# qitianwu/SGFormer

Measured on AMD Instinct MI355X. Metric: SGFormer fwd+bwd nodes/sec on ogbn-products full-graph, higher is better.
Workload: dtype bf16

## Files before the change

include/sgf.h:

```cpp
#ifndef SGF_H_
#define SGF_H_

#include <stddef.h>
#include <stdint.h>

#ifdef __cplusplus
extern "C" {
#endif

#define SGF_VERSION 666

#define SGF_F32 0
#define SGF_BF16 1
#define SGF_F32_BF16X3 2

#define SGF_OK 0
#define SGF_E_INVALID (-1)
#define SGF_E_WORKSPACE (-2)
#define SGF_E_HIP (-3)
#define SGF_E_UNSUPPORTED (-4)

int sgf_version(void);
const char* sgf_last_error(void);
int sgf_reload_env(void);

size_t sgf_csr_workspace_bytes(int64_t nnz, int64_t n);
int sgf_csr_build(const int64_t* edge_index, int64_t nnz, int64_t n, int64_t* rowptr,
                  int32_t* colind, float* val, int32_t* deg, void* workspace,
                  size_t workspace_bytes, void* stream);

int sgf_csr_transpose(const int64_t* edge_index, int64_t nnz, int64_t n, const int32_t* deg,
                      const int64_t* rowptr, const int32_t* colind, int64_t* t_rowptr,
                      int32_t* t_colind, float* t_val, int32_t* is_symmetric, void* workspace,
                      size_t workspace_bytes, void* stream);

size_t sgf_subgraph_workspace_bytes(int64_t nnz, int64_t n);
int sgf_subgraph_plan(const int64_t* edge_index, int64_t nnz, int64_t n, const int64_t* subset,
                      int64_t m, int32_t* relabel, int64_t* total, void* workspace,
                      size_t workspace_bytes, void* stream);
int sgf_subgraph_emit(const int64_t* edge_index, int64_t nnz, int64_t n, const int32_t* relabel,
                      int32_t relabel_nodes, int64_t total, int64_t* out, int64_t* out_eid,
                      void* workspace, size_t workspace_bytes, void* stream);

// ... 353 lines not shown
size_t sgf_argmax_workspace_bytes(int64_t m, int32_t c);
int sgf_argmax_count(const void* logits, int64_t ldl, int64_t n, int32_t c, int32_t dtype, const void* labels,
                     int64_t label_stride, int32_t label_kind, const int64_t* idx, int64_t m, int64_t* counts,
                     void* workspace, size_t workspace_bytes, void* stream);

int32_t sgf_head_rows_supported(int32_t d, int32_t classes, int32_t dtype);
size_t sgf_head_rows_fwd_workspace_bytes(int64_t m);
size_t sgf_head_rows_bwd_workspace_bytes(int64_t m, int32_t d, int32_t classes);
int sgf_head_rows_fwd(const void* x1, int64_t ld1, float a, const void* x2, int64_t ld2, float b, const float* w,
                      const float* bias, int64_t n, int32_t d, int32_t classes, int32_t dtype, const int64_t* idx,
                      int64_t m, float* logits, int64_t ldl, const int64_t* labels, float* lse, float* loss_sum,
                      int64_t* counts, void* workspace, size_t workspace_bytes, void* stream);
int sgf_head_rows_bwd(const void* x1, int64_t ld1, float a, const void* x2, int64_t ld2, float b, const float* w,
                      int64_t n, int32_t d, int32_t classes, int32_t dtype, const int64_t* idx, int64_t m,
                      const float* dlogits, int64_t lddl, const float* logits, int64_t ldl, const float* lse,
                      const int64_t* labels, const float* gout, float inv_denom, void* dx1, int64_t ldd1, void* dx2,
                      int64_t ldd2, float* dw, float* db, void* workspace, size_t workspace_bytes, void* stream);

int32_t sgf_pair_sigmoid_supported(int32_t heads, int32_t v_heads, int32_t d, int32_t dtype);
size_t sgf_pair_sigmoid_workspace_bytes(int64_t n, int64_t l, int32_t heads);
int64_t sgf_pair_sigmoid_lap_rows(int32_t which, int32_t heads, int32_t d, int32_t dtype, int32_t laps);
int sgf_pair_sigmoid_fwd(const void* q, int64_t ldq, const void* k, int64_t ldk, const void* v, int64_t ldv, int64_t n,
                         int64_t l, int32_t heads, int32_t v_heads, int32_t d, int32_t dtype, void* out, int64_t ldo,
                         float* rowsum, void* stream);
int sgf_pair_sigmoid_bwd_q(const void* g, int64_t ldg, const void* out, int64_t ldo, const float* rowsum, const void* q,
                           int64_t ldq, const void* k, int64_t ldk, const void* v, int64_t ldv, int64_t n, int64_t l,
                           int32_t heads, int32_t v_heads, int32_t d, int32_t dtype, void* dq, int64_t lddq, void* workspace,
                           size_t workspace_bytes, void* stream);
int sgf_pair_sigmoid_bwd_kv(const void* g, int64_t ldg, const float* rowsum, const void* q, int64_t ldq, const void* k,
                            int64_t ldk, const void* v, int64_t ldv, int64_t n, int64_t l, int32_t heads, int32_t v_heads,
                            int32_t d, int32_t dtype, void* dk, int64_t lddk, void* dv, int64_t lddv, const void* workspace,
                            size_t workspace_bytes, void* stream);

int sgf_sum_n(const void* const* xs_host, const int64_t* lds_host, int32_t k, int64_t n, int32_t d,
              int32_t dtype, void* y, int64_t ldy, void* stream);

size_t sgf_colsum_workspace_bytes(int64_t n, int32_t d);
int sgf_colsum(const void* x, int64_t ldx, int64_t n, int32_t d, int32_t dtype, float* out,
               void* workspace, size_t workspace_bytes, void* stream);

int32_t sgf_comm_available(void);
int32_t sgf_comm_unique_id_bytes(void);
int sgf_comm_unique_id(void* id_host);
int sgf_comm_create(void** comm_out, int32_t world, int32_t rank, const void* id_host);
int sgf_comm_destroy(void* comm);
int sgf_comm_all_reduce_f32(void* comm, float* buf, int64_t count, void* stream);
int sgf_comm_all_gather(void* comm, const void* send, void* recv, int64_t bytes_per_rank, void* stream);
int sgf_comm_all_to_all(void* comm, const void* send, const int64_t* send_offset_host, const int64_t* send_bytes_host,
                        void* recv, const int64_t* recv_offset_host, const int64_t* recv_bytes_host, void* stream);

#ifdef __cplusplus
}
#endif
#endif
```

sgformer_amd/_lib.py:

```python
from __future__ import annotations

import ctypes
import os
from ctypes import c_char_p, c_double, c_float, c_int32, c_int64, c_size_t, c_uint64, c_void_p

_HERE = os.path.dirname(os.path.abspath(__file__))
LIB_PATH = os.path.join(_HERE, "lib", "libsgf.so")

SGF_F32 = 0
SGF_BF16 = 1
SGF_F32_BF16X3 = 2
SGF_OK = 0
SGF_E_INVALID = -1
SGF_E_WORKSPACE = -2
SGF_E_HIP = -3
SGF_E_UNSUPPORTED = -4
SGF_BCE_TARGET_F32 = 0
SGF_BCE_TARGET_I64 = 1
SGF_BCE_TARGET_CLASS = 2
SGF_METRIC_TARGET_F32 = 0
SGF_METRIC_TARGET_I64 = 1

_lib = None

# ... 144 lines not shown
                                  c_int64, _P]),
    "sgf_nll_workspace_bytes": (c_size_t, [c_int64]),
    "sgf_nll_fwd": (c_int32, [_P, c_int64, c_int64, c_int32, c_int32, _P, _P, c_int64, _P, _P, c_size_t, _P]),
    "sgf_nll_bwd": (c_int32, [_P, c_int64, c_int64, c_int32, c_int32, _P, _P, c_int64, _P, c_float, _P,
                              c_int64, _P]),
    "sgf_bce_workspace_bytes": (c_size_t, [c_int64, c_int32]),
    "sgf_bce_fwd": (c_int32, [_P, c_int64, c_int64, c_int32, c_int32, _P, c_int64, c_int32, _P, c_int64, c_float, _P, _P,
                              c_size_t, _P]),
    "sgf_bce_bwd": (c_int32, [_P, c_int64, c_int64, c_int32, c_int32, _P, c_int64, c_int32, _P, c_int64, _P, c_float, _P,
                              c_int64, _P]),
    "sgf_rocauc_workspace_bytes": (c_size_t, [c_int64, c_int32]),
    "sgf_rocauc_counts": (c_int32, [_P, c_int64, c_int64, c_int32, c_int32, _P, c_int64, c_int32, _P, c_int64, _P, _P,
                                    c_size_t, _P]),
    "sgf_argmax_workspace_bytes": (c_size_t, [c_int64, c_int32]),
    "sgf_argmax_count": (c_int32, [_P, c_int64, c_int64, c_int32, c_int32, _P, c_int64, c_int32, _P, c_int64, _P, _P,
                                   c_size_t, _P]),
    "sgf_head_rows_supported": (c_int32, [c_int32, c_int32, c_int32]),
    "sgf_head_rows_fwd_workspace_bytes": (c_size_t, [c_int64]),
    "sgf_head_rows_bwd_workspace_bytes": (c_size_t, [c_int64, c_int32, c_int32]),
    "sgf_head_rows_fwd": (c_int32, [_P, c_int64, c_float, _P, c_int64, c_float, _P, _P, c_int64, c_int32, c_int32, c_int32,
                                    _P, c_int64, _P, c_int64, _P, _P, _P, _P, _P, c_size_t, _P]),
    "sgf_head_rows_bwd": (c_int32, [_P, c_int64, c_float, _P, c_int64, c_float, _P, c_int64, c_int32, c_int32, c_int32,
                                    _P, c_int64, _P, c_int64, _P, c_int64, _P, _P, _P, c_float, _P, c_int64, _P, c_int64,
                                    _P, _P, _P, c_size_t, _P]),
    "sgf_pair_sigmoid_supported": (c_int32, [c_int32, c_int32, c_int32, c_int32]),
    "sgf_pair_sigmoid_workspace_bytes": (c_size_t, [c_int64, c_int64, c_int32]),
    "sgf_pair_sigmoid_lap_rows": (c_int64, [c_int32, c_int32, c_int32, c_int32, c_int32]),
    "sgf_pair_sigmoid_fwd": (c_int32, [_P, c_int64, _P, c_int64, _P, c_int64, c_int64, c_int64, c_int32, c_int32, c_int32,
                                       c_int32, _P, c_int64, _P, _P]),
    "sgf_pair_sigmoid_bwd_q": (c_int32, [_P, c_int64, _P, c_int64, _P, _P, c_int64, _P, c_int64, _P, c_int64, c_int64,
                                         c_int64, c_int32, c_int32, c_int32, c_int32, _P, c_int64, _P, c_size_t, _P]),
    "sgf_pair_sigmoid_bwd_kv": (c_int32, [_P, c_int64, _P, _P, c_int64, _P, c_int64, _P, c_int64, c_int64, c_int64, c_int32,
                                          c_int32, c_int32, c_int32, _P, c_int64, _P, c_int64, _P, c_size_t, _P]),
    "sgf_sum_n": (c_int32, [_P, _P, c_int32, c_int64, c_int32, c_int32, _P, c_int64, _P]),
    "sgf_colsum_workspace_bytes": (c_size_t, [c_int64, c_int32]),
    "sgf_colsum": (c_int32, [_P, c_int64, c_int64, c_int32, c_int32, _P, _P, c_size_t, _P]),
    "sgf_combine_fc_supported": (c_int32, [c_int32, c_int32, c_int32]),
    "sgf_combine_fc_fwd": (c_int32, [_P, c_int64, c_float, _P, c_int64, c_float, _P, _P, c_int64, c_int32, c_int32,
                                     c_int32, _P, c_int64, _P]),
    "sgf_combine_fc_bwd": (c_int32, [_P, c_int64, _P, c_int64, c_int32, c_int32, c_float, c_float, c_int32, _P,
                                     c_int64, _P, c_int64, _P]),
    "sgf_combine_fc_fwd_mapped": (c_int32, [_P, c_int64, c_float, _P, c_int64, c_float, _P, _P, c_int64, c_int32, c_int32,
                                     c_int32, _P, c_int64, _P, _P]),
    "sgf_combine_fc_bwd_g": (c_int32, [_P, c_int64, _P, c_int64, c_int32, c_int32, c_float, c_float, c_int32, _P, c_int64, _P,
                                       c_int64, _P, _P, c_int64, _P]),
    "sgf_combine_fc_bwd_mapped": (c_int32, [_P, c_int64, _P, c_int64, c_int32, c_int32, c_float, c_float, c_int32, _P,
                                     c_int64, _P, c_int64, _P, _P]),
    "sgf_gcn_epilogue_supported": (c_int32, [c_int32, c_int32, c_int32]),
    "sgf_gcn_epilogue_workspace_bytes": (c_size_t, [c_int64, c_int32]),
    "sgf_gcn_epilogue_stats": (c_int32, [_P, c_int64, _P, c_int64, _P, c_int64, c_int32, c_int32, c_int32, _P, c_int64,
                                         _P, _P, _P, c_size_t, _P]),
    "sgf_gcn_epilogue_dx": (c_int32, [_P, c_int64, _P, c_int64, c_int64, c_int32, c_int32, c_int32, _P, c_int64, _P]),
    "sgf_gcn_epilogue_dx2": (c_int32, [_P, c_int64, _P, _P, c_int64, c_int64, c_int32, c_int32, _P, c_int64, _P, c_int64,
                                       c_int32, _P]),
    "sgf_gcn_epilogue_dx2_acc_supported": (c_int32, [c_int32, c_int32]),
    "sgf_gcn_epilogue_dx2_acc": (c_int32, [_P, c_int64, _P, c_int64, c_int64, c_int32, c_int32, _P, c_int64, _P, c_int64, _P,
                                           c_int64, _P, c_int64, _P]),
    "sgf_gcn_epilogue_apply": (c_int32, [_P, c_int64, _P, _P, _P, _P, _P, c_int64, c_int32, c_int64, c_int32,
                               c_int32, _P, c_int64, _P]),
    "sgf_gcn_bn_bwd_dx_supported": (c_int32, [c_int32, c_int32]),
    "sgf_gcn_bn_bwd_dx_workspace_bytes": (c_size_t, [c_int64, c_int32]),
    "sgf_gcn_bn_bwd_dx": (c_int32, [_P, c_int64, _P, c_int64, _P, _P, _P, _P, c_int32, _P, c_float, c_int32, _P, c_int64,
                                    c_int64, c_int32, c_int32, _P, c_int64, _P, c_int64, _P, _P, c_size_t, _P, c_int64,
                                    c_int32, _P, c_size_t, _P]),
    "sgf_gcn_epilogue_cat_supported": (c_int32, [c_int32, c_int32]),
    "sgf_gcn_epilogue_cat": (c_int32, [_P, c_int64, _P, c_int64, _P, c_int64, _P, c_int64, c_int32, c_int32, _P, c_int64,
# ... 62 lines not shown
```

sgformer_amd/csrc/fused.hip:

```cpp
#include "common.h"

namespace sgf {
namespace {

constexpr int kThreads = 256;
constexpr int kMaxD = 1024;
constexpr int kMaxStatBlocks = 2048;

__device__ __forceinline__ float4 zero4() { return make_float4(0.f, 0.f, 0.f, 0.f); }
__device__ __forceinline__ float4 ld4f(const float* p) { return *reinterpret_cast<const float4*>(p); }

inline int lanes_per_row(int d) {
  int l = 16;
  while (l * 4 < d && l < 64) l <<= 1;
  return l;
}

template <typename T, int LPR, int NC>
__global__ __launch_bounds__(kThreads) void k_ln_fwd(
    const T* __restrict__ x, int64_t ldx, const T* __restrict__ res, int64_t ldr, float a, float b,
    const float* __restrict__ gamma, const float* __restrict__ beta, int relu, float eps, int64_t n,
    int d, T* __restrict__ y, int64_t ldy, float* __restrict__ mean, float* __restrict__ rstd) {
  constexpr int RPB = kThreads / LPR;
  const int sl = threadIdx.x % LPR;
// ... 831 lines not shown
      }
    };
    int64_t row = r0 + sr;
    for (; row + (U - 1) * static_cast<int64_t>(rpp) < r1; row += U * static_cast<int64_t>(rpp)) {
      uint4 xv[U], gv[U], hv[U];
#pragma unroll
      for (int u = 0; u < U; ++u) {
        const int64_t rr = row + u * static_cast<int64_t>(rpp);
        xv[u] = *reinterpret_cast<const uint4*>(x + rr * ldx + col);
        gv[u] = *reinterpret_cast<const uint4*>(dy + rr * lddy + col);
        if (kTwo) hv[u] = *reinterpret_cast<const uint4*>(dy2 + rr * lddy2 + col);
      }
#pragma unroll
      for (int u = 0; u < U; ++u) add_row(xv[u], gv[u], kTwo ? hv[u] : gv[u]);
    }
    for (; row < r1; row += rpp) {
      const uint4 xr = *reinterpret_cast<const uint4*>(x + row * ldx + col);
      const uint4 gr = *reinterpret_cast<const uint4*>(dy + row * lddy + col);
      const uint4 hr = kTwo ? *reinterpret_cast<const uint4*>(dy2 + row * lddy2 + col) : gr;
      add_row(xr, gr, hr);
    }
  }
#pragma unroll
  for (int e = 0; e < 8; ++e) {
    red[(0 * kThreads + threadIdx.x) * 8 + e] = s0[e];
    red[(1 * kThreads + threadIdx.x) * 8 + e] = s1[e];
  }
  __syncthreads();
  for (int j = threadIdx.x; j < 2 * d; j += kThreads) {
    const int which = j / d, cc = j % d;
    float s = 0.f;
    for (int r = 0; r < rpp; ++r) s += red[(which * kThreads + r * f8 + cc / 8) * 8 + (cc & 7)];
    part[static_cast<int64_t>(blockIdx.x) * 2 * d + j] = s;
  }
}

template <typename T>
__global__ __launch_bounds__(kThreads) void k_axpby(const T* __restrict__ x1, int64_t ld1, float a,
                                                    const T* __restrict__ x2, int64_t ld2, float b,
                                                    int64_t n, int d, T* __restrict__ y,
                                                    int64_t ldy) {
  const int f4 = d / 4;
  const int64_t total = n * f4;
  for (int64_t i = static_cast<int64_t>(blockIdx.x) * kThreads + threadIdx.x; i < total;
       i += static_cast<int64_t>(gridDim.x) * kThreads) {
    const int64_t row = i / f4;
    const int col = static_cast<int>(i % f4) * 4;
    const float4 u = load4<T>(x1 + row * ld1 + col);
    const float4 v = load4<T>(x2 + row * ld2 + col);
    store4<T>(y + row * ldy + col,
              make_float4(a * u.x + b * v.x, a * u.y + b * v.y, a * u.z + b * v.z, a * u.w + b * v.w));
  }
}

template <typename TS, typename TD, typename TI>
__global__ __launch_bounds__(kThreads) void k_gather_rows(const TS* __restrict__ src, int64_t lds,
                                                          const TI* __restrict__ idx, int64_t n_out, int d,
                                                          int64_t n_src, TD* __restrict__ dst, int64_t ldd,
                                                          int vec) {
  if (vec) {
    const int f4 = d / 4;
    const int64_t total = n_out * f4;
    for (int64_t i = static_cast<int64_t>(blockIdx.x) * kThreads + threadIdx.x; i < total;
         i += static_cast<int64_t>(gridDim.x) * kThreads) {
      const int64_t row = i / f4;
      const int col = static_cast<int>(i % f4) * 4;
// ... 599 lines not shown
}

extern "C" int sgf_bn_bwd_stats(const void* dy, int64_t lddy, const void* x, int64_t ldx,
                                const float* mean, const float* rstd, const float* gamma,
                                const float* beta, int32_t relu, int64_t n, int32_t d,
                                int32_t dtype, float* stats, void* workspace,
                                size_t workspace_bytes, void* stream) {
  return sgf_bn_bwd_stats2(dy, lddy, nullptr, 0, x, ldx, mean, rstd, gamma, beta, relu, n, d, dtype, stats, workspace,
                           workspace_bytes, stream);
}

extern "C" int sgf_bn_bwd_apply(const void* dy, int64_t lddy, const void* x, int64_t ldx,
                                const float* mean, const float* rstd, const float* gamma,
                                const float* beta, int32_t relu, const float* stats, float inv_n,
                                int32_t training, int64_t n, int32_t d, int32_t dtype, void* dx,
                                int64_t lddx, void* stream) {
  int rc = check_ew("sgf_bn_bwd_apply", n, d, dtype);
  if (rc != SGF_OK || n == 0) return rc;
  SGF_REQUIRE(dy && x && dx && mean && rstd && (!training || stats), SGF_E_INVALID,
              "sgf_bn_bwd_apply: null pointer");
  SGF_REQUIRE(lddy % 4 == 0 && ldx % 4 == 0 && lddx % 4 == 0, SGF_E_INVALID,
              "sgf_bn_bwd_apply: leading dims must be multiples of 4");
  hipStream_t st = static_cast<hipStream_t>(stream);
  const BnParams p{mean, rstd, gamma, beta};
  if (dtype == SGF_BF16 && ew8_rows(d, {{dy, lddy}, {x, ldx}, {dx, lddx}}))
    return launch(k_bn_bwd_apply_bf16x8<kEw8Unroll>, dim3(rowwalk8_grid(n, d)), st, dy, lddy, x, ldx, p, relu, stats, inv_n,
                  training, n, d, dx, lddx);
  return by_dtype(dtype, [&](auto t) {
    return launch(k_bn_bwd_apply<decltype(t)>, dim3(rowwalk_grid(n, d)), st, dy, lddy, x, ldx, p, relu, stats, inv_n, training,
                  n, d, dx, lddx);
  });
}

extern "C" int sgf_axpby(const void* x1, int64_t ld1, float a, const void* x2, int64_t ld2, float b,
                         int64_t n, int32_t d, int32_t dtype, void* y, int64_t ldy, void* stream) {
  int rc = check_ew("sgf_axpby", n, d, dtype);
  if (rc != SGF_OK || n == 0) return rc;
  SGF_REQUIRE(x1 && x2 && y && ld1 % 4 == 0 && ld2 % 4 == 0 && ldy % 4 == 0, SGF_E_INVALID,
              "sgf_axpby: bad pointer / ld");
  hipStream_t st = static_cast<hipStream_t>(stream);
  return by_dtype(dtype, [&](auto t) {
    return launch(k_axpby<decltype(t)>, dim3(ew_grid(n * (d / 4))), st, x1, ld1, a, x2, ld2, b, n, d, y, ldy);
  });
}

extern "C" int sgf_gather_rows(const void* src, int64_t lds, int32_t src_dtype, int64_t n_src, const void* idx,
                               int32_t idx_is_int64, int64_t n_out, int32_t d, void* dst, int64_t ldd,
                               int32_t dst_dtype, void* stream) {
  SGF_REQUIRE(n_out >= 0 && d >= 0 && n_src >= 0, SGF_E_INVALID, "sgf_gather_rows: negative size");
  SGF_REQUIRE((src_dtype == SGF_F32 || src_dtype == SGF_BF16) && (dst_dtype == SGF_F32 || dst_dtype == SGF_BF16),
              SGF_E_INVALID, "sgf_gather_rows: unknown dtype");
  if (n_out == 0 || d == 0) return SGF_OK;
  SGF_REQUIRE(src && idx && dst && lds >= d && ldd >= d, SGF_E_INVALID, "sgf_gather_rows: bad pointer / ld");
  const size_t es = src_dtype == SGF_BF16 ? 2 : 4, ed = dst_dtype == SGF_BF16 ? 2 : 4;
  const int vec = d % 4 == 0 && lds % 4 == 0 && ldd % 4 == 0 && reinterpret_cast<uintptr_t>(src) % (4 * es) == 0 &&
                  reinterpret_cast<uintptr_t>(dst) % (4 * ed) == 0;
  hipStream_t st = static_cast<hipStream_t>(stream);
  const dim3 grid(ew_grid(vec ? n_out * (d / 4) : n_out * d));
  return by_copy_types(src_dtype, dst_dtype, idx_is_int64, [&](auto ts, auto td, auto ti) {
    return launch(k_gather_rows<decltype(ts), decltype(td), decltype(ti)>, grid, st, src, lds, idx, n_out, d, n_src, dst, ldd,
                  vec);
  });
}

namespace sgf {
namespace {
// ... 170 lines not shown
```

sgformer_amd/linear.py:

```python
from __future__ import annotations

import os
from functools import partial
from typing import NamedTuple, Optional

import torch
import torch.nn.functional as F

from .kernels import _pair_gram, _rows, _rows16

_F32 = torch.float32
_BF16 = torch.bfloat16

from .graph import K, _has


def _f32c(t):
    return None if t is None else t.detach().float().contiguous()


def _switch(name: str, default: bool) -> bool:
    v = os.environ.get(name)
    return default if v is None else (v != "0" if default else v == "1")

# ... 307 lines not shown

def gcn_layer_fused_ok(x0: torch.Tensor, w: torch.Tensor) -> bool:
    d = x0.shape[1] if x0.dim() == 2 else 0
    return (x0.dim() == 2 and x0.shape[0] > 0 and x0.dtype == _BF16 and tuple(w.shape) == (d, 2 * d)
            and _has(K, "gcn_bn_bwd_dx_supported", d, x0.dtype) and _switch("SGF_GCN_FUSED", True))


class _LinearBNActRes(torch.autograd.Function):

    @staticmethod
    def forward(ctx, y, x0, w, b, gamma, beta, book, relu: bool, use_res: bool, shard, chain, first: bool, pack=None):
        K.check(y, x0)
        dt = x0.dtype
        wc = w.detach().to(dt).contiguous()
        yr, xr = _rows16(y), _rows16(x0)
        z, mean, rstd, n_tot, training = _batchnorm_of(book, partial(_streaming_linear, [yr, xr], wc, _f32c(b)), wc.shape[0],
                                                       yr.shape[0], yr.device, shard)
        g32, be32 = _f32c(gamma), _f32c(beta)
        if pack is not None:
            out, pack["out"] = K.bn_apply_packed(z, mean, rstd, g32, be32, xr if use_res else None, relu, pack["slot_bytes"])
        else:
            out = K.bn_apply(z, mean, rstd, g32, be32, xr if use_res else None, relu)
        ctx.save_for_backward(yr, xr, z, wc, g32, be32, mean, rstd)
        ctx.meta = (bool(relu), bool(use_res), bool(training), float(n_tot), shard, chain, bool(first), w.dtype,
                    None if b is None else b.dtype, None if gamma is None else gamma.dtype)
        return out

    @staticmethod
    def backward(ctx, gout):
        yr, xr, z, wc, g32, be32, mean, rstd = ctx.saved_tensors
        relu, use_res, training, n_tot, shard, chain, first, wdt, bdt, gdt = ctx.meta
        d = z.shape[1]
        gout = _rows16(gout.contiguous())
        stats = K.bn_bwd_stats(gout, z, mean, rstd, g32, be32, relu)
        if shard is not None:
            shard.all_reduce(stats)
        inv_n = 1.0 / max(n_tot, 1.0)
        if _fused_bwd():
            dz, dy, acc = K.gcn_bn_bwd_dx(gout, z, mean, rstd, g32, be32, relu, stats, inv_n, training, wc, chain.acc,
                                          last=first, add_gy=use_res)
            chain.acc = None if first else acc
            dx0 = acc if first else None
        else:
            fused_dw = None
            if ctx.needs_input_grad[2] and _pair_gram() and _has(K, "gram2_bn_bwd_supported", gout, z, yr, xr):
                dwf = torch.empty((d, 2 * d), dtype=_F32, device=z.device)
                dz, dbf = K.gram2_bn_bwd(gout, z, mean, rstd, g32, be32, relu, stats, inv_n, training, yr, xr, dwf[:, :d], dwf[:, d:])
                fused_dw = (dwf.to(wdt), dbf.to(bdt) if (ctx.needs_input_grad[3] and bdt is not None) else None)
            else:
                dz = K.bn_bwd_apply(gout, z, mean, rstd, g32, be32, relu, stats, inv_n, training)
            if _acc_in_place(d, dz.dtype) and not chain.parts:
                dy, chain.acc = K.gcn_epilogue_dx2_acc(dz, wc, _rows16(gout) if use_res else None, chain.acc)
                dx0 = None
                if first:
                    dx0, chain.acc = chain.acc, None
            else:
                dy, dxi = K.gcn_epilogue_dx2(dz, wc[:, :d], wc[:, d:], True)
                chain.parts.append(dxi)
                if use_res:
                    chain.parts.append(gout)
                dx0 = None
                if first:
                    parts, chain.parts = chain.parts, []
                    if chain.acc is not None:
                        parts.append(chain.acc)
                        chain.acc = None
                    dx0 = parts[0] if len(parts) == 1 else (K.sum_n(parts) if len(parts) <= 8 else sum(parts[1:], parts[0]))
        if not _fused_bwd() and fused_dw is not None:
            dw, db = fused_dw
        else:
            dw, db = _linear_param_grads(dz, [yr, xr], [d, d], ctx.needs_input_grad[2],
                                         ctx.needs_input_grad[3] and bdt is not None, wdt, bdt)
        dgamma, dbeta = _bn_param_grads(stats, d, g32, be32, gdt, shard)
        return dy, dx0, dw, db, dgamma, dbeta, None, None, None, None, None, None, None


def linear_bn_act_res(y, x0, w, b, gamma, beta, book, relu, use_res, shard, chain, first, pack=None):
    return _LinearBNActRes.apply(y, x0, w, b, gamma, beta, book, relu, use_res, shard, chain, first, pack)


def _linear(w, b, *xs):
# ... 38 lines not shown
```

sgformer_amd/ops.py:

```python
from __future__ import annotations

from typing import Optional

import torch
import torch.nn.functional as F

from . import kernels as _kernels
from .kernels import HipKernels, LONG_ROW, _SEGMENT, _workspace
from .kernels import _rows, _rows16

_F32 = torch.float32
_BF16 = torch.bfloat16


from . import graph as _graph
from .graph import *
from .graph import K, graph_cache, _own_block_spmm, _sharded_spmm, _tile_params, _block_shape, _mode
from .linear import _bn_param_grads, _f32c, _has, _switch


def set_kernels(table):
    global K
    prev, K = K, table
    _graph.K = _linear.K = table
    graph_cache.clear()
    return prev


def _require_cuda(*tensors):
    K.check(*tensors)


def _split(qkv, v_ext, heads, d):
    hd = heads * d
    q, k = qkv[:, :hd], qkv[:, hd:2 * hd]
    if v_ext is None:
        return q, k, qkv[:, 2 * hd:], heads
    return q, k, v_ext, 1


class _Attention(torch.autograd.Function):

    @staticmethod
    def forward(ctx, qkv, v_ext, heads: int, d: int, shard, n_override=None, per_head=False):
        K.check(qkv, v_ext)
        qkv, v_ext = _rows(qkv), _rows(v_ext)
        n, hd = qkv.shape[0], heads * d
        assert qkv.shape[1] == (3 * hd if v_ext is None else 2 * hd)
        q, k, v, v_heads = _split(qkv, v_ext, heads, d)
        stats = K.attn_fwd_reduce(q, k, v, heads, v_heads, d)
        n_total = float(n) if n_override is None else float(n_override)
        if shard is not None:
            shard.all_reduce(stats)
            if n_override is None:
                n_total = float(shard.n_global)
        out, den, o_heads = K.attn_fwd_apply(q, v, stats, n_total, heads, v_heads, d)
        per_head = bool(per_head) and heads > 1
        ctx.save_for_backward(qkv, v_ext, out, den, o_heads, stats)
        ctx.meta = (heads, d, n_total, shard, per_head)
        return o_heads if per_head else out

    @staticmethod
    def backward(ctx, g):
# ... 180 lines not shown
        return g, None


def grad_tap(x, holder):
    if not (torch.is_grad_enabled() and x.requires_grad):
        return x
    return _GradTap.apply(x, holder)


def attention_stats(q: torch.Tensor, k: torch.Tensor, v: torch.Tensor):
    K.check(q, k, v)
    n, heads, d = q.shape
    q2, k2, v2 = (_rows(t.reshape(n, -1)) for t in (q, k, v))
    return K.attn_fwd_reduce(q2, k2, v2, heads, v.shape[1], d)


class _LNResAct(torch.autograd.Function):
    @staticmethod
    def forward(ctx, x, res, a: float, b: float, gamma, beta, relu: bool, eps: float):
        K.check(x, res, gamma)
        x, res = _rows(x), _rows(res)
        has_ln = gamma is not None
        g32, b32 = (_f32c(gamma), _f32c(beta)) if has_ln else (None, None)
        y, mean, rstd = K.ln_fwd(x, res, a, b, g32, b32, relu, eps)
        ctx.save_for_backward(x, res, y if relu else None, g32, mean, rstd)
        ctx.meta = (float(a), float(b), bool(relu), gamma.dtype if has_ln else None)
        return y

    @staticmethod
    def backward(ctx, gy):
        x, res, y, g32, mean, rstd = ctx.saved_tensors
        a, b, relu, pdtype = ctx.meta
        gy = _rows(gy.contiguous())
        dx, dres, dgamma, dbeta = K.ln_bwd(gy, y, x, res, a, b, g32, relu, mean, rstd)
        if g32 is not None:
            dgamma, dbeta = dgamma.to(pdtype), dbeta.to(pdtype)
        return dx, dres, None, None, dgamma, dbeta, None, None


def ln_res_act(x, res, a, b, gamma, beta, relu, eps=1e-5):
    return _LNResAct.apply(x, res, a, b, gamma, beta, relu, eps)


class _BNActRes(torch.autograd.Function):
    @staticmethod
    def forward(ctx, x, res, gamma, beta, mean, rstd, relu: bool, training: bool, n_tot: float,
                shard):
        K.check(x, res)
        x, res = _rows(x), _rows(res)
        g32, b32, mean, rstd = _f32c(gamma), _f32c(beta), _f32c(mean), _f32c(rstd)
        y = K.bn_apply(x, mean, rstd, g32, b32, res, relu)
        ctx.save_for_backward(x, g32, b32, mean, rstd)
        ctx.meta = (bool(relu), bool(training), float(n_tot), shard, res is not None,
                    gamma.dtype if gamma is not None else None)
        return y

    @staticmethod
    def backward(ctx, gy):
        x, g32, b32, mean, rstd = ctx.saved_tensors
        relu, training, n_tot, shard, has_res, pdtype = ctx.meta
        gy = _rows(gy.contiguous())
        d = x.shape[1]
        stats = K.bn_bwd_stats(gy, x, mean, rstd, g32, b32, relu)
        if shard is not None:
            shard.all_reduce(stats)
        dx = K.bn_bwd_apply(gy, x, mean, rstd, g32, b32, relu, stats, 1.0 / max(n_tot, 1.0), training)
        dgamma, dbeta = _bn_param_grads(stats, d, g32, b32, pdtype, shard)
# ... 20 lines not shown
        ctx.meta = (float(p), seed, res is not None)
        return K.dropout(x, res, p, seed)

    @staticmethod
    def backward(ctx, gy):
        p, seed, has_res = ctx.meta
        gy = _rows(gy.contiguous())
        if isinstance(seed, tuple):
            return K.dropout_dev(gy, None, p, seed[0], seed[1]), (gy if has_res else None), None
        return K.dropout(gy, None, p, seed), (gy if has_res else None), None


def dropout_res(x, res, p: float):
    return _DropoutRes.apply(x, res, p)


class _NllRows(torch.autograd.Function):
    @staticmethod
    def forward(ctx, logits, labels, idx, denom):
        K.check(logits, labels, idx)
        logits = logits if logits.stride(-1) == 1 else logits.contiguous()
        labels = labels.reshape(-1).contiguous()
        idx = idx.contiguous()
        if idx.dtype == torch.bool:
            idx = idx.nonzero().view(-1)
        m = idx.numel() if denom is None else denom
        ctx.save_for_backward(logits, labels, idx)
        ctx.inv = 1.0 / float(max(m, 1))
        return (K.nll_fwd(logits, labels, idx) * ctx.inv).reshape(())

    @staticmethod
    def backward(ctx, g):
        logits, labels, idx = ctx.saved_tensors
        return K.nll_bwd(logits, labels, idx, g.reshape(1).float().contiguous(), ctx.inv), None, None, None


def nll_loss_rows(logits, labels, idx, denom=None):
    return _NllRows.apply(logits, labels, idx, denom)


def _bce_target(logits, target):
    n, c = logits.shape
    if target.shape == logits.shape:
        if target.dtype in (_F32, torch.int64):
            return target if target.is_contiguous() else target.contiguous()
        if target.is_floating_point() or target.dtype == torch.bool:
            return target.to(_F32).contiguous()
        if not target.is_complex():
            return target.to(torch.int64).contiguous()
    elif (c > 1 and target.numel() == n and target.shape in ((n,), (n, 1)) and not target.is_floating_point()
          and not target.is_complex() and target.dtype != torch.bool):
        return target.reshape(-1).to(torch.int64).contiguous()
    raise ValueError(f"bce_loss_rows: cannot read a {target.dtype} target of shape {tuple(target.shape)} for logits "
                     f"{tuple(logits.shape)}: pass a [N, C] multi-hot / soft target, or integer class indices [N] or [N, 1] "
                     "(C > 1)")


class _BceRows(torch.autograd.Function):
    @staticmethod
    def forward(ctx, logits, target, idx, denom):
        K.check(logits, target, idx)
        if logits.dim() != 2:
            raise ValueError(f"bce_loss_rows: logits must be [N, C], got {tuple(logits.shape)}")
        n, c = logits.shape
        if logits.stride(1) != 1 or (logits.stride(0) < c and n > 1):
            logits = logits.contiguous()
        target = _bce_target(logits, target)
# ... 115 lines not shown
        return ga, (ga if a == b else g * b), None, None


def axpby(x1, x2, a, b):
    return _Axpby.apply(x1, x2, a, b)


class _CombineFC(torch.autograd.Function):
    @staticmethod
    def forward(ctx, x1, x2, w, bias, a: float, b: float, row_map=None):
        K.check(x1, x2)
        x1, x2 = _rows16(x1), _rows16(x2)
        ctx.row_map = row_map
        w32, b32 = _f32c(w), _f32c(bias)
        c = w32.shape[0]
        if (x1.dtype == _F32 or c > 64) and c % 4 != 0:
            w32, b32 = F.pad(w32, (0, 0, 0, 4 - c % 4)), F.pad(b32, (0, 4 - c % 4))
        ctx.save_for_backward(x1, x2, w32)
        ctx.meta = (float(a), float(b), w.dtype, bias.dtype, c)
        out = K.combine_fc_fwd(x1, a, x2, b, w32, b32) if row_map is None else K.combine_fc_fwd(x1, a, x2, b, w32, b32, row_map)
        return out if out.shape[1] == c else out[:, :c]

    @staticmethod
    def backward(ctx, g):
        x1, x2, w32 = ctx.saved_tensors
        a, b, wdtype, bdtype, c = ctx.meta
        g = g.float()
        if w32.shape[0] != g.shape[1]:
            g = F.pad(g, (0, w32.shape[0] - g.shape[1]))
        g = g.contiguous()
        row_map = ctx.row_map
        if x1.dtype == _BF16 and _has(K, "combine_fc_bwd_g") and g.shape[1] <= 64:
            dx1, dx2, gp = K.combine_fc_bwd_g(g, w32, a, b, row_map)
        else:
            dx1, dx2 = K.combine_fc_bwd(g, w32, a, b, x1.dtype) if row_map is None else K.combine_fc_bwd(g, w32, a, b, x1.dtype,
                                                                                                           row_map)
            gp = K.gather_rows(g, row_map, x1.dtype) if row_map is not None else g.to(x1.dtype)
            if gp.shape[1] % 4 != 0:
                gp = F.pad(gp, (0, 4 - gp.shape[1] % 4))
            gp = _rows(gp)
        dw1, db = K.gram(gp, x1, want_colsum=True)
        dw2, _ = K.gram(gp, x2, want_colsum=False)
        return dx1, dx2, (a * dw1 + b * dw2)[:c].to(wdtype), db[:c].to(bdtype), None, None, None


def combine_fc(x1, x2, w, bias, a: float, b: float, row_map=None) -> torch.Tensor:
    return _CombineFC.apply(x1, x2, w, bias, a, b, row_map)


def combine_fc_mapped_supported(x: torch.Tensor, classes: int) -> bool:
    return (x.dim() == 2 and _switch("SGF_HEAD_MAPPED", True)
            and _has(K, "combine_fc_mapped_supported", x.shape[1], classes, x.dtype))


def combine_fc_supported(x: torch.Tensor, classes: int) -> bool:
    if x.dim() == 2 and x.dtype == _BF16 and classes > 64 and not _switch("SGF_HEAD_WIDE", False):
        return False
    return x.dim() == 2 and K.combine_fc_supported(x.shape[1], classes, x.dtype)



from . import linear as _linear
from .linear import *
from .linear import (_BN_SAMPLE_ROWS, _Linear, _LinearBNActRes, _StemPair, _StemPairBN, _acc_in_place, _fused_bwd, _linear_param_grads,
                     _linear_with_stats, _streaming_linear, _streaming_linear_ok)
```

Before: 29.69 million.

## Propagate a live-row bitmap from the loss to skip dead-row gradient reads

Builds a bitmap of the rows selected by the training loss index and carries it through autograd from the NLL backward, via the combine-FC head backward, into the BatchNorm and LayerNorm backward kernels. New bf16 d=256 kernels skip loading the upstream gradient for rows known to have zero gradient, which cuts memory traffic when only a subset of nodes (e.g. training split) contributes to the loss. This relies on a pointer-keyed registry and version checks to decide when the mask is still valid. A stale or mismatched mask would silently produce wrong gradients.

```diff
diff --git a/include/sgf.h b/include/sgf.h
--- a/include/sgf.h
+++ b/include/sgf.h
@@ -8,7 +8,7 @@
 extern "C" {
 #endif
 
-#define SGF_VERSION 666
+#define SGF_VERSION 667
 
 #define SGF_F32 0
 #define SGF_BF16 1
@@ -428,6 +428,20 @@
                             int32_t d, int32_t dtype, void* dk, int64_t lddk, void* dv, int64_t lddv, const void* workspace,
                             size_t workspace_bytes, void* stream);
 
+int32_t sgf_live_rows_supported(int32_t d, int32_t classes, int32_t dtype);
+int sgf_live_rows_build(const int64_t* idx, int64_t m, int64_t n, uint32_t* live, void* stream);
+int sgf_bn_bwd_stats_live(const void* dy, int64_t lddy, const void* x, int64_t ldx, const float* mean, const float* rstd,
+                          const float* gamma, const float* beta, int32_t relu, int64_t n, int32_t d, int32_t dtype,
+                          const uint32_t* live, float* stats, void* workspace, size_t workspace_bytes, void* stream);
+int sgf_bn_bwd_apply_live(const void* dy, int64_t lddy, const void* x, int64_t ldx, const float* mean, const float* rstd,
+                          const float* gamma, const float* beta, int32_t relu, const float* stats, float inv_n,
+                          int32_t training, int64_t n, int32_t d, int32_t dtype, const uint32_t* live, void* dx,
+                          int64_t lddx, void* stream);
+int sgf_ln_bwd_live(const void* dy, int64_t lddy, const void* y, int64_t ldy, const void* x, int64_t ldx, const void* res,
+                    int64_t ldr, float a, float b, const float* gamma, int32_t relu, const float* mean, const float* rstd,
+                    int64_t n, int32_t d, int32_t dtype, const uint32_t* live, void* dx, int64_t lddx, void* dres,
+                    int64_t lddres, float* dgamma, float* dbeta, void* workspace, size_t workspace_bytes, void* stream);
+
 int sgf_sum_n(const void* const* xs_host, const int64_t* lds_host, int32_t k, int64_t n, int32_t d,
               int32_t dtype, void* y, int64_t ldy, void* stream);
 
diff --git a/sgformer_amd/_lib.py b/sgformer_amd/_lib.py
--- a/sgformer_amd/_lib.py
+++ b/sgformer_amd/_lib.py
@@ -200,6 +200,14 @@
                                          c_int64, c_int32, c_int32, c_int32, c_int32, _P, c_int64, _P, c_size_t, _P]),
     "sgf_pair_sigmoid_bwd_kv": (c_int32, [_P, c_int64, _P, _P, c_int64, _P, c_int64, _P, c_int64, c_int64, c_int64, c_int32,
                                           c_int32, c_int32, c_int32, _P, c_int64, _P, c_int64, _P, c_size_t, _P]),
+    "sgf_live_rows_supported": (c_int32, [c_int32, c_int32, c_int32]),
+    "sgf_live_rows_build": (c_int32, [_P, c_int64, c_int64, _P, _P]),
+    "sgf_bn_bwd_stats_live": (c_int32, [_P, c_int64, _P, c_int64, _P, _P, _P, _P, c_int32, c_int64, c_int32, c_int32, _P, _P,
+                                        _P, c_size_t, _P]),
+    "sgf_bn_bwd_apply_live": (c_int32, [_P, c_int64, _P, c_int64, _P, _P, _P, _P, c_int32, _P, c_float, c_int32, c_int64,
+                                        c_int32, c_int32, _P, _P, c_int64, _P]),
+    "sgf_ln_bwd_live": (c_int32, [_P, c_int64, _P, c_int64, _P, c_int64, _P, c_int64, c_float, c_float, _P, c_int32, _P, _P,
+                                  c_int64, c_int32, c_int32, _P, _P, c_int64, _P, c_int64, _P, _P, _P, c_size_t, _P]),
     "sgf_sum_n": (c_int32, [_P, _P, c_int32, c_int64, c_int32, c_int32, _P, c_int64, _P]),
     "sgf_colsum_workspace_bytes": (c_size_t, [c_int64, c_int32]),
     "sgf_colsum": (c_int32, [_P, c_int64, c_int64, c_int32, c_int32, _P, _P, c_size_t, _P]),
diff --git a/sgformer_amd/csrc/fused.hip b/sgformer_amd/csrc/fused.hip
--- a/sgformer_amd/csrc/fused.hip
+++ b/sgformer_amd/csrc/fused.hip
@@ -887,6 +887,265 @@
     float s = 0.f;
     for (int r = 0; r < rpp; ++r) s += red[(which * kThreads + r * f8 + cc / 8) * 8 + (cc & 7)];
     part[static_cast<int64_t>(blockIdx.x) * 2 * d + j] = s;
+  }
+}
+
+constexpr int kLiveD = 256;
+
+template <int U>
+__device__ __forceinline__ uint32_t live_bits(const uint32_t* __restrict__ live, int64_t row, int stride, int64_t end) {
+  uint32_t m = 0;
+#pragma unroll
+  for (int u = 0; u < U; ++u) {
+    const int64_t rr = row + static_cast<int64_t>(u) * stride;
+    if (rr < end) m |= ((live[rr >> 5] >> (rr & 31)) & 1u) << u;
+  }
+  return m;
+}
+
+template <int U>
+__global__ __launch_bounds__(kThreads) void k_bn_bwd_stats_live_bf16x8(
+    const uint16_t* __restrict__ dy, int64_t lddy, const uint16_t* __restrict__ x, int64_t ldx, BnParams p, int relu, int64_t n,
+    const uint32_t* __restrict__ live, float* __restrict__ part) {
+  constexpr int d = kLiveD, f8 = d / 8, rpp = kThreads / f8;
+  __shared__ float red[2 * kThreads * 8];
+  const int c8 = threadIdx.x % f8;
+  const int sr = threadIdx.x / f8;
+  const int col = c8 * 8;
+  float s0[8], s1[8];
+#pragma unroll
+  for (int e = 0; e < 8; ++e) s0[e] = s1[e] = 0.f;
+  BnCoeffs8 c;
+  bn_coeffs8(p, col, c);
+  const int64_t rows_per_blk = (n + gridDim.x - 1) / gridDim.x;
+  const int64_t r0 = static_cast<int64_t>(blockIdx.x) * rows_per_blk;
+  int64_t r1 = r0 + rows_per_blk;
+  if (r1 > n) r1 = n;
+  uint32_t lv = live_bits<U>(live, r0 + sr, rpp, r1);
+  for (int64_t row = r0 + sr; row < r1; row += U * static_cast<int64_t>(rpp)) {
+    const uint32_t nx = live_bits<U>(live, row + U * static_cast<int64_t>(rpp), rpp, r1);
+    uint4 xv[U], gv[U];
+#pragma unroll
+    for (int u = 0; u < U; ++u) {
+      if ((lv >> u) & 1u) {
+        const int64_t rr = row + u * static_cast<int64_t>(rpp);
+        xv[u] = *reinterpret_cast<const uint4*>(x + rr * ldx + col);
+        gv[u] = *reinterpret_cast<const uint4*>(dy + rr * lddy + col);
+      }
+    }
+#pragma unroll
+    for (int u = 0; u < U; ++u) {
+      if ((lv >> u) & 1u) {
+        float v[8], g[8];
+        ew_unpack(xv[u], v);
+        ew_unpack(gv[u], g);
+#pragma unroll
+        for (int e = 0; e < 8; ++e) {
+          float ge = g[e];
+          const float xh = (v[e] - c.mu[e]) * c.rs[e];
+          if (relu) ge = fmaf(xh, c.ga[e], c.be[e]) > 0.f ? ge : 0.f;
+          s0[e] += ge;
+          s1[e] += ge * xh;
+        }
+      }
+    }
+    lv = nx;
+  }
+#pragma unroll
+  for (int e = 0; e < 8; ++e) {
+    red[(0 * kThreads + threadIdx.x) * 8 + e] = s0[e];
+    red[(1 * kThreads + threadIdx.x) * 8 + e] = s1[e];
+  }
+  __syncthreads();
+  for (int j = threadIdx.x; j < 2 * d; j += kThreads) {
+    const int which = j / d, cc = j % d;
+    float s = 0.f;
+    for (int r = 0; r < rpp; ++r) s += red[(which * kThreads + r * f8 + cc / 8) * 8 + (cc & 7)];
+    part[static_cast<int64_t>(blockIdx.x) * 2 * d + j] = s;
+  }
+}
+
+template <int U>
+__global__ __launch_bounds__(kThreads) void k_bn_bwd_apply_live_bf16x8(
+    const uint16_t* __restrict__ dy, int64_t lddy, const uint16_t* __restrict__ x, int64_t ldx, BnParams p, int relu,
+    const float* __restrict__ stats, float inv_n, int training, int64_t n, const uint32_t* __restrict__ live,
+    uint16_t* __restrict__ dx, int64_t lddx) {
+  constexpr int d = kLiveD, f8 = d / 8, rpp = kThreads / f8;
+  const int sr = threadIdx.x / f8;
+  const int col = (threadIdx.x % f8) * 8;
+  BnCoeffs8 c;
+  bn_coeffs8(p, col, c);
+  float s0[8], s1[8];
+#pragma unroll
+  for (int e = 0; e < 8; ++e) {
+    s0[e] = training ? stats[col + e] : 0.f;
+    s1[e] = training ? stats[d + col + e] : 0.f;
+  }
+  const int64_t rpb = static_cast<int64_t>(rpp) * U;
+  const int64_t lap = static_cast<int64_t>(gridDim.x) * rpb;
+  int64_t row0 = static_cast<int64_t>(blockIdx.x) * rpb + sr;
+  uint32_t lv = live_bits<U>(live, row0, rpp, n);
+  for (; row0 < n; row0 += lap) {
+    const uint32_t nx = live_bits<U>(live, row0 + lap, rpp, n);
+    uint4 xv[U], gv[U];
+#pragma unroll
+    for (int u = 0; u < U; ++u) {
+      const int64_t row = row0 + u * rpp;
+      gv[u] = make_uint4(0u, 0u, 0u, 0u);
+      if (row < n) {
+        xv[u] = *reinterpret_cast<const uint4*>(x + row * ldx + col);
+        if ((lv >> u) & 1u) gv[u] = *reinterpret_cast<const uint4*>(dy + row * lddy + col);
+      }
+    }
+#pragma unroll
+    for (int u = 0; u < U; ++u) {
+      const int64_t row = row0 + u * rpp;
+      if (row < n) {
+        float v[8], g[8], o[8];
+        ew_unpack(xv[u], v);
+        ew_unpack(gv[u], g);
+#pragma unroll
+        for (int e = 0; e < 8; ++e) {
+          const float xh = (v[e] - c.mu[e]) * c.rs[e];
+          float ge = g[e];
+          if (relu) ge = fmaf(xh, c.ga[e], c.be[e]) > 0.f ? ge : 0.f;
+          if (training) ge -= s0[e] * inv_n + xh * s1[e] * inv_n;
+          o[e] = c.ga[e] * c.rs[e] * ge;
+        }
+        *reinterpret_cast<uint4*>(dx + row * lddx + col) = ew_pack8(o);
+      }
+    }
+    lv = nx;
+  }
+}
+
+template <int R>
+__global__ __launch_bounds__(kThreads) void k_ln_bwd_live_bf16x8(
+    const uint16_t* __restrict__ dy, int64_t lddy, const uint16_t* __restrict__ y, int64_t ldy, const uint16_t* __restrict__ x,
+    int64_t ldx, const uint16_t* __restrict__ res, int64_t ldr, float a, float b, const float* __restrict__ gamma, int relu,
+    const float* __restrict__ mean, const float* __restrict__ rstd, int64_t n, const uint32_t* __restrict__ live,
+    uint16_t* __restrict__ dxo, int64_t lddx, uint16_t* __restrict__ dro, int64_t lddr, float* __restrict__ part) {
+  constexpr int LPR = kLiveD / 8;
+  constexpr int RPS = kThreads / LPR;
+  constexpr int RPB = RPS * R;
+  constexpr int D = kLiveD;
+  constexpr float inv_d = 1.0f / static_cast<float>(D);
+  static_assert(RPB == 32, "one mask word per block trip");
+  __shared__ float red[2 * RPS * D];
+  const int sl = threadIdx.x % LPR;
+  const int sr = threadIdx.x / LPR;
+  const int col = sl * 8;
+  const bool ln = gamma != nullptr;
+  float gm[8], dg[8], db[8];
+#pragma unroll
+  for (int e = 0; e < 8; ++e) {
+    gm[e] = ln ? gamma[col + e] : 1.f;
+    dg[e] = db[e] = 0.f;
+  }
+  const int64_t lap = static_cast<int64_t>(gridDim.x) * RPB;
+  int64_t row0 = static_cast<int64_t>(blockIdx.x) * RPB;
+  uint32_t word = row0 < n ? live[row0 >> 5] : 0u;
+  for (; row0 < n; row0 += lap) {
+    const uint32_t nxt = row0 + lap < n ? live[(row0 + lap) >> 5] : 0u;
+    uint4 gv[R], yv[R], xv[R], rv[R];
+    float mu[R], rs[R];
+#pragma unroll
+    for (int q = 0; q < R; ++q) {
+      const int64_t row = row0 + q * RPS + sr;
+      gv[q] = yv[q] = xv[q] = rv[q] = make_uint4(0u, 0u, 0u, 0u);
+      mu[q] = 0.f;
+      rs[q] = ln ? 0.f : 1.f;
+      if (row < n && ((word >> (q * RPS + sr)) & 1u)) {
+        gv[q] = *reinterpret_cast<const uint4*>(dy + row * lddy + col);
+        if (relu) yv[q] = *reinterpret_cast<const uint4*>(y + row * ldy + col);
+        if (ln) {
+          xv[q] = *reinterpret_cast<const uint4*>(x + row * ldx + col);
+          if (res) rv[q] = *reinterpret_cast<const uint4*>(res + row * ldr + col);
+          mu[q] = mean[row];
+          rs[q] = rstd[row];
+        }
+      }
+    }
+#pragma unroll
+    for (int q = 0; q < R; ++q) {
+      const int64_t row = row0 + q * RPS + sr;
+      const bool rok = row < n;
+      float g[8], h[8];
+      ew_unpack(gv[q], g);
+      if (relu) {
+        float yy[8];
+        ew_unpack(yv[q], yy);
+#pragma unroll
+        for (int e = 0; e < 8; ++e) g[e] = yy[e] > 0.f ? g[e] : 0.f;
+      }
+      float s1 = 0.f, s2 = 0.f;
+      if (ln) {
+        float v[8];
+        ew_unpack(xv[q], v);
+#pragma unroll
+        for (int e = 0; e < 8; ++e) v[e] *= a;
+        if (res) {
+          float r[8];
+          ew_unpack(rv[q], r);
+#pragma unroll
+          for (int e = 0; e < 8; ++e) v[e] = fmaf(b, r[e], v[e]);
+        }
+#pragma unroll
+        for (int e = 0; e < 8; ++e) {
+          h[e] = (v[e] - mu[q]) * rs[q];
+          if (rok) {
+            dg[e] += g[e] * h[e];
+            db[e] += g[e];
+          }
+          g[e] *= gm[e];
+          s1 += g[e];
+          s2 += g[e] * h[e];
+        }
+      } else {
+#pragma unroll
+        for (int e = 0; e < 8; ++e) h[e] = 0.f;
+      }
+      float m1 = 0.f, m2 = 0.f;
+      if (ln) {
+        m1 = group_sum<LPR>(s1) * inv_d;
+        m2 = group_sum<LPR>(s2) * inv_d;
+      }
+      if (rok) {
+        float o[8], o2[8];
+#pragma unroll
+        for (int e = 0; e < 8; ++e) {
+          const float dp = ln ? rs[q] * (g[e] - m1 - h[e] * m2) : g[e];
+          o[e] = a * dp;
+          o2[e] = b * dp;
+        }
+        *reinterpret_cast<uint4*>(dxo + row * lddx + col) = ew_pack8(o);
+        if (dro != nullptr) *reinterpret_cast<uint4*>(dro + row * lddr + col) = ew_pack8(o2);
+      }
+    }
+    word = nxt;
+  }
+  if (!ln) return;
+#pragma unroll
+  for (int e = 0; e < 8; ++e) {
+    red[(0 * RPS + sr) * D + col + e] = dg[e];
+    red[(1 * RPS + sr) * D + col + e] = db[e];
+  }
+  __syncthreads();
+  for (int j = threadIdx.x; j < 2 * D; j += kThreads) {
+    const int which = j / D, cc = j % D;
+    float s = 0.f;
+    for (int r = 0; r < RPS; ++r) s += red[(which * RPS + r) * D + cc];
+    part[static_cast<int64_t>(blockIdx.x) * 2 * D + j] = s;
+  }
+}
+
+__global__ __launch_bounds__(kThreads) void k_live_rows_build(const int64_t* __restrict__ idx, int64_t m, int64_t n,
+                                                              uint32_t* __restrict__ live) {
+  for (int64_t i = static_cast<int64_t>(blockIdx.x) * kThreads + threadIdx.x; i < m;
+       i += static_cast<int64_t>(gridDim.x) * kThreads) {
+    int64_t r = idx[i];
+    if (r < 0) r += n;
+    if (r >= 0 && r < n) atomicOr(&live[r >> 5], 1u << (r & 31));
   }
 }
 
@@ -1552,6 +1811,90 @@
   });
 }
 
+extern "C" int32_t sgf_live_rows_supported(int32_t d, int32_t classes, int32_t dtype) {
+  return dtype == SGF_BF16 && d == kLiveD && classes >= 1 && classes <= 64 && ew8_rows(kLiveD, {}) ? 1 : 0;
+}
+
+extern "C" int sgf_live_rows_build(const int64_t* idx, int64_t m, int64_t n, uint32_t* live, void* stream) {
+  SGF_REQUIRE(n >= 0 && m >= 0, SGF_E_INVALID, "sgf_live_rows_build: bad sizes");
+  if (n == 0) return SGF_OK;
+  SGF_REQUIRE(live && (idx || m == 0), SGF_E_INVALID, "sgf_live_rows_build: null pointer");
+  hipStream_t st = static_cast<hipStream_t>(stream);
+  SGF_CHECK_HIP(hipMemsetAsync(live, 0, static_cast<size_t>((n + 31) / 32) * sizeof(uint32_t), st));
+  if (m == 0) return SGF_OK;
+  return launch(k_live_rows_build, dim3(clamp_grid(ceil_div(m, static_cast<int64_t>(kThreads)))), st, idx, m, n, live);
+}
+
+namespace {
+int check_live(const char* fn, int64_t n, int d, int dtype, const uint32_t* live,
+               std::initializer_list<std::pair<const void*, int64_t>> ops) {
+  int rc = check_ew(fn, n, d, dtype);
+  if (rc != SGF_OK) return rc;
+  SGF_REQUIRE(dtype == SGF_BF16 && d == kLiveD, SGF_E_UNSUPPORTED, "%s: bf16 rows of %d columns only (d=%d)", fn, kLiveD, d);
+  SGF_REQUIRE(n == 0 || live, SGF_E_INVALID, "%s: null live mask (call the dense entry)", fn);
+  SGF_REQUIRE(n == 0 || rows16(ops), SGF_E_INVALID, "%s: rows must be 16-byte aligned", fn);
+  return SGF_OK;
+}
+}
+
+extern "C" int sgf_bn_bwd_stats_live(const void* dy, int64_t lddy, const void* x, int64_t ldx, const float* mean,
+                                     const float* rstd, const float* gamma, const float* beta, int32_t relu, int64_t n,
+                                     int32_t d, int32_t dtype, const uint32_t* live, float* stats, void* workspace,
+                                     size_t workspace_bytes, void* stream) {
+  const char* fn = "sgf_bn_bwd_stats_live";
+  int rc = check_live(fn, n, d, dtype, live, {{dy, lddy}, {x, ldx}});
+  if (rc != SGF_OK) return rc;
+  hipStream_t st = static_cast<hipStream_t>(stream);
+  SGF_REQUIRE(stats, SGF_E_INVALID, "%s: null stats", fn);
+  if (n == 0) return zero_floats(stats, 2 * d, st);
+  SGF_REQUIRE(dy && x && mean && rstd, SGF_E_INVALID, "%s: null pointer", fn);
+  SGF_REQUIRE(workspace && workspace_bytes >= sgf_colstats_workspace_bytes(n, d), SGF_E_WORKSPACE, "%s: workspace too small", fn);
+  const BnParams p{mean, rstd, gamma, beta};
+  const int nblk = stat_blocks(n);
+  rc = launch(k_bn_bwd_stats_live_bf16x8<kEw8Unroll>, dim3(nblk), st, dy, lddy, x, ldx, p, relu, n, live, workspace);
+  return rc != SGF_OK ? rc : sum_partials(static_cast<float*>(workspace), nblk, 2 * d, stats, stats + d, d, st);
+}
+
+extern "C" int sgf_bn_bwd_apply_live(const void* dy, int64_t lddy, const void* x, int64_t ldx, const float* mean,
+                                     const float* rstd, const float* gamma, const float* beta, int32_t relu,
+                                     const float* stats, float inv_n, int32_t training, int64_t n, int32_t d, int32_t dtype,
+                                     const uint32_t* live, void* dx, int64_t lddx, void* stream) {
+  const char* fn = "sgf_bn_bwd_apply_live";
+  int rc = check_live(fn, n, d, dtype, live, {{dy, lddy}, {x, ldx}, {dx, lddx}});
+  if (rc != SGF_OK || n == 0) return rc;
+  SGF_REQUIRE(dy && x && dx && mean && rstd && (!training || stats), SGF_E_INVALID, "%s: null pointer", fn);
+  const BnParams p{mean, rstd, gamma, beta};
+  return launch(k_bn_bwd_apply_live_bf16x8<kEw8Unroll>, dim3(rowwalk8_grid(n, d)), static_cast<hipStream_t>(stream), dy, lddy,
+                x, ldx, p, relu, stats, inv_n, training, n, live, dx, lddx);
+}
+
+extern "C" int sgf_ln_bwd_live(const void* dy, int64_t lddy, const void* y, int64_t ldy, const void* x, int64_t ldx,
+                               const void* res, int64_t ldr, float a, float b, const float* gamma, int32_t relu,
+                               const float* mean, const float* rstd, int64_t n, int32_t d, int32_t dtype,
+                               const uint32_t* live, void* dx, int64_t lddx, void* dres, int64_t lddres, float* dgamma,
+                               float* dbeta, void* workspace, size_t workspace_bytes, void* stream) {
+  const char* fn = "sgf_ln_bwd_live";
+  int rc = check_live(fn, n, d, dtype, live,
+                      {{dy, lddy}, {relu ? y : nullptr, ldy}, {gamma ? x : nullptr, ldx}, {gamma ? res : nullptr, ldr},
+                       {dx, lddx}, {dres, lddres}});
+  if (rc != SGF_OK) return rc;
+  hipStream_t st = static_cast<hipStream_t>(stream);
+  if (n == 0) {
+    if (gamma && dgamma && (rc = zero_floats(dgamma, d, st)) != SGF_OK) return rc;
+    return gamma && dbeta ? zero_floats(dbeta, d, st) : SGF_OK;
+  }
+  SGF_REQUIRE(dy && dx && (!relu || y) && (!gamma || (x && mean && rstd)), SGF_E_INVALID, "%s: null pointer", fn);
+  SGF_REQUIRE(!gamma || (workspace && workspace_bytes >= sgf_ln_bwd_workspace_bytes(n, d)), SGF_E_WORKSPACE,
+              "%s: workspace too small", fn);
+  constexpr int R = 4;
+  const int nblk = clamp_grid(ceil_div(n, kThreads / (d / 8) * R), kMaxStatBlocks);
+  float* part = static_cast<float*>(workspace);
+  rc = launch(k_ln_bwd_live_bf16x8<R>, dim3(nblk), st, dy, lddy, y, ldy, x, ldx, res, ldr, a, b, gamma, relu, mean, rstd, n,
+              live, dx, lddx, dres, lddres, part);
+  if (rc != SGF_OK || !gamma || !(dgamma || dbeta)) return rc;
+  return sum_partials(part, nblk, 2 * d, dgamma, dbeta, d, st);
+}
+
 extern "C" int sgf_axpby(const void* x1, int64_t ld1, float a, const void* x2, int64_t ld2, float b,
                          int64_t n, int32_t d, int32_t dtype, void* y, int64_t ldy, void* stream) {
   int rc = check_ew("sgf_axpby", n, d, dtype);
diff --git a/sgformer_amd/linear.py b/sgformer_amd/linear.py
--- a/sgformer_amd/linear.py
+++ b/sgformer_amd/linear.py
@@ -363,7 +363,12 @@
         relu, use_res, training, n_tot, shard, chain, first, wdt, bdt, gdt = ctx.meta
         d = z.shape[1]
         gout = _rows16(gout.contiguous())
-        stats = K.bn_bwd_stats(gout, z, mean, rstd, g32, be32, relu)
+        from . import live_rows
+        live = live_rows.bn_bwd(gout, z, shard)
+        if live is not None:
+            stats = live_rows.bn_bwd_stats(gout, z, mean, rstd, g32, be32, relu, live)
+        else:
+            stats = K.bn_bwd_stats(gout, z, mean, rstd, g32, be32, relu)
         if shard is not None:
             shard.all_reduce(stats)
         inv_n = 1.0 / max(n_tot, 1.0)
@@ -378,6 +383,8 @@
                 dwf = torch.empty((d, 2 * d), dtype=_F32, device=z.device)
                 dz, dbf = K.gram2_bn_bwd(gout, z, mean, rstd, g32, be32, relu, stats, inv_n, training, yr, xr, dwf[:, :d], dwf[:, d:])
                 fused_dw = (dwf.to(wdt), dbf.to(bdt) if (ctx.needs_input_grad[3] and bdt is not None) else None)
+            elif live is not None:
+                dz = live_rows.bn_bwd_apply(gout, z, mean, rstd, g32, be32, relu, stats, inv_n, training, live)
             else:
                 dz = K.bn_bwd_apply(gout, z, mean, rstd, g32, be32, relu, stats, inv_n, training)
             if _acc_in_place(d, dz.dtype) and not chain.parts:
diff --git a/sgformer_amd/live_rows.py b/sgformer_amd/live_rows.py
--- /dev/null
+++ b/sgformer_amd/live_rows.py
@@ -0,0 +1,159 @@
+from __future__ import annotations
+
+import torch
+
+from . import _lib, ops
+from .kernels import _code, _ld, _launch, _scratch
+from .linear import _switch
+
+_F32 = torch.float32
+_BF16 = torch.bfloat16
+
+
+def enabled() -> bool:
+    return _switch("SGF_LIVE_ROWS", True)
+
+
+class _Hip:
+    @staticmethod
+    def live_rows_supported(d: int, classes: int, dtype) -> bool:
+        return dtype == _BF16 and bool(_lib.load().sgf_live_rows_supported(int(d), int(classes), _lib.SGF_BF16))
+
+    @staticmethod
+    def live_rows_build(idx, n: int) -> torch.Tensor:
+        live = torch.empty((n + 31) // 32, dtype=torch.int32, device=idx.device)
+        _launch(idx.device, "sgf_live_rows_build", idx, idx.numel(), n, live)
+        return live
+
+    @staticmethod
+    def bn_bwd_stats_live(gy, x, mean, rstd, gamma, beta, relu: bool, live) -> torch.Tensor:
+        n, d = x.shape
+        dev = x.device
+        stats = torch.empty(2 * d, dtype=_F32, device=dev)
+        _launch(dev, "sgf_bn_bwd_stats_live", gy, _ld(gy), x, _ld(x), mean, rstd, gamma, beta, int(relu), n, d, _code(x), live,
+                stats, *_scratch(dev, "col", _lib.load().sgf_colstats_workspace_bytes(n, d)))
+        return stats
+
+    @staticmethod
+    def bn_bwd_apply_live(gy, x, mean, rstd, gamma, beta, relu: bool, stats, inv_n: float, training: bool, live):
+        n, d = x.shape
+        dx = torch.empty_like(x)
+        _launch(x.device, "sgf_bn_bwd_apply_live", gy, _ld(gy), x, _ld(x), mean, rstd, gamma, beta, int(relu), stats,
+                float(inv_n), int(training), n, d, _code(x), live, dx, _ld(dx))
+        return dx
+
+    @staticmethod
+    def ln_bwd_live(gy, y, x, res, a: float, b: float, gamma, relu: bool, mean, rstd, live):
+        n, d = x.shape
+        dev = x.device
+        dx = torch.empty_like(x)
+        shared = res is not None and float(a) == float(b)
+        dres = torch.empty_like(res) if (res is not None and not shared) else None
+        dgamma = torch.empty(d, dtype=_F32, device=dev) if gamma is not None else None
+        dbeta = torch.empty(d, dtype=_F32, device=dev) if gamma is not None else None
+        _launch(dev, "sgf_ln_bwd_live", gy, _ld(gy), y, _ld(y), x, _ld(x), res, _ld(res), float(a), float(b), gamma, int(relu),
+                mean, rstd, n, d, _code(x), live, dx, _ld(dx), dres, _ld(dres), dgamma, dbeta,
+                *_scratch(dev, "ln", _lib.load().sgf_ln_bwd_workspace_bytes(n, d)))
+        return dx, (dx if shared else dres), dgamma, dbeta
+
+
+def _table():
+    k = ops.K
+    if hasattr(k, "live_rows_build"):
+        return k
+    return _Hip if k.name == "hip" else None
+
+
+def _capturing() -> bool:
+    return torch.cuda.is_available() and torch.cuda.is_current_stream_capturing()
+
+
+_registry: "dict[int, tuple]" = {}
+_MAX_ENTRIES = 8
+
+
+def clear():
+    _registry.clear()
+
+
+def register(t: torch.Tensor, live: torch.Tensor):
+    if len(_registry) >= _MAX_ENTRIES:
+        _registry.pop(next(iter(_registry)))
+    _registry[t.data_ptr()] = (t.detach(), tuple(t.shape), t.stride(), t._version, live)
+
+
+def take(t) -> "torch.Tensor | None":
+    if t is None or not _registry:
+        return None
+    hit = _registry.pop(t.data_ptr(), None)
+    if hit is None:
+        return None
+    alias, shape, stride, version, live = hit
+    if (t._is_view() or tuple(t.shape) != shape or t.stride() != stride or t._version != version or t.dtype != alias.dtype
+            or t.untyped_storage().data_ptr() != alias.untyped_storage().data_ptr()):
+        return None
+    if live.is_cuda:
+        live.record_stream(torch.cuda.current_stream(live.device))
+    return live
+
+
+def usable(x, classes: int, shard=None) -> bool:
+    if not enabled() or shard is not None or x.dim() != 2 or _capturing():
+        return False
+    k = _table()
+    return k is not None and bool(k.live_rows_supported(x.shape[1], classes, x.dtype))
+
+
+_BITMAPS: "dict[tuple, tuple]" = {}
+
+
+def _bitmap_of(k, idx, n: int) -> torch.Tensor:
+    key = (idx.data_ptr(), idx._version, idx.numel(), int(n), str(idx.device))
+    hit = _BITMAPS.get(key)
+    if hit is None:
+        if len(_BITMAPS) >= 4:
+            _BITMAPS.pop(next(iter(_BITMAPS)))
+        _BITMAPS[key] = hit = (k.live_rows_build(idx, n), idx)
+    return hit[0]
+
+
+def from_loss(dlogits: torch.Tensor, idx: torch.Tensor):
+    clear()
+    if not enabled() or dlogits.dim() != 2 or dlogits.shape[1] > 64 or idx.dtype != torch.int64 or _capturing():
+        return
+    k = _table()
+    if k is None:
+        return
+    register(dlogits, _bitmap_of(k, idx.contiguous(), dlogits.shape[0]))
+    try:
+        torch.autograd.Variable._execution_engine.queue_callback(clear)
+    except RuntimeError:
+        pass
+
+
+def head_bwd(g, dx1, dx2, x1, row_map):
+    live = take(g)
+    if live is None or row_map is not None or not usable(x1, g.shape[1]):
+        return
+    register(dx1, live)
+    register(dx2, live)
+
+
+def bn_bwd(gout, z, shard):
+    live = take(gout)
+    return live if (live is not None and usable(z, 1, shard)) else None
+
+
+def bn_bwd_stats(gout, z, mean, rstd, gamma, beta, relu, live):
+    return _table().bn_bwd_stats_live(gout, z, mean, rstd, gamma, beta, relu, live)
+
+
+def bn_bwd_apply(gout, z, mean, rstd, gamma, beta, relu, stats, inv_n, training, live):
+    return _table().bn_bwd_apply_live(gout, z, mean, rstd, gamma, beta, relu, stats, inv_n, training, live)
+
+
+def ln_bwd(gy, y, x, res, a, b, gamma, relu, mean, rstd):
+    live = take(gy)
+    if live is None or not usable(x, 1):
+        return None
+    return _table().ln_bwd_live(gy, y, x, res, a, b, gamma, relu, mean, rstd, live)
diff --git a/sgformer_amd/ops.py b/sgformer_amd/ops.py
--- a/sgformer_amd/ops.py
+++ b/sgformer_amd/ops.py
@@ -29,6 +29,11 @@
 
 def _require_cuda(*tensors):
     K.check(*tensors)
+
+
+def _live_rows():
+    from . import live_rows
+    return live_rows
 
 
 def _split(qkv, v_ext, heads, d):
@@ -275,7 +280,8 @@
         x, res, y, g32, mean, rstd = ctx.saved_tensors
         a, b, relu, pdtype = ctx.meta
         gy = _rows(gy.contiguous())
-        dx, dres, dgamma, dbeta = K.ln_bwd(gy, y, x, res, a, b, g32, relu, mean, rstd)
+        dx, dres, dgamma, dbeta = (_live_rows().ln_bwd(gy, y, x, res, a, b, g32, relu, mean, rstd)
+                                   or K.ln_bwd(gy, y, x, res, a, b, g32, relu, mean, rstd))
         if g32 is not None:
             dgamma, dbeta = dgamma.to(pdtype), dbeta.to(pdtype)
         return dx, dres, None, None, dgamma, dbeta, None, None
@@ -362,7 +368,9 @@
     @staticmethod
     def backward(ctx, g):
         logits, labels, idx = ctx.saved_tensors
-        return K.nll_bwd(logits, labels, idx, g.reshape(1).float().contiguous(), ctx.inv), None, None, None
+        d = K.nll_bwd(logits, labels, idx, g.reshape(1).float().contiguous(), ctx.inv)
+        _live_rows().from_loss(d, idx)
+        return d, None, None, None
 
 
 def nll_loss_rows(logits, labels, idx, denom=None):
@@ -544,6 +552,7 @@
         row_map = ctx.row_map
         if x1.dtype == _BF16 and _has(K, "combine_fc_bwd_g") and g.shape[1] <= 64:
             dx1, dx2, gp = K.combine_fc_bwd_g(g, w32, a, b, row_map)
+            _live_rows().head_bwd(g, dx1, dx2, x1, row_map)
         else:
             dx1, dx2 = K.combine_fc_bwd(g, w32, a, b, x1.dtype) if row_map is None else K.combine_fc_bwd(g, w32, a, b, x1.dtype,
                                                                                                            row_map)
```

Result: slower. 29.30 million (-1.3%).
